# joshspeagle/frankenz

Measured on AMD Instinct MI355X. Metric: object-template likelihood evals/sec (fused fit_predict -> PDFs), higher is better.
Workload: dtype f64 throughout (chi2, ln-likes, every weight, ln-evidence, PDFs; an fp32 estimate of the weight only CLASSIFIES which pairs can matter to an fp64 sum, DESIGN.md 3.1)

## Files before the change

### frankenz_amd/csrc/fz_hist.h

```cpp
#pragma once
#include <type_traits>
#include "fz_kernels.h"
#include "fz_nolist.h"

namespace fz {

#define FZ_HEXP_K 256
#ifndef FZ_HIST_MP
#define FZ_HIST_MP 1
#endif
#ifndef FZ_HIST_TILE384
#define FZ_HIST_TILE384 1
#endif
#ifndef FZ_HIST_REFRESH_TILE
#define FZ_HIST_REFRESH_TILE 1
#endif
#ifndef FZ_HIST_STAGE_LATE
#define FZ_HIST_STAGE_LATE 1
#endif
#ifndef FZ_HIST_SETTLE2
#define FZ_HIST_SETTLE2 0
#endif
#ifndef FZ_HIST_SEG_NW0
#define FZ_HIST_SEG_NW0 16
#endif
#ifndef FZ_HIST_SEG_PFMAX
#define FZ_HIST_SEG_PFMAX 12
#endif
#ifndef FZ_HIST_REFRESH
#define FZ_HIST_REFRESH 32
#endif
#ifndef FZ_HIST_LEAN
#define FZ_HIST_LEAN 1
#endif
#ifndef FZ_HIST_AHEAD
#define FZ_HIST_AHEAD 1
#endif
template <bool L>
__device__ __forceinline__ double fma3(double a, double b, double c) {
    if constexpr (L) { double d; asm("v_fma_f64 %0, %1, %2, %3" : "=v"(d) : "v"(a), "v"(b), "v"(c)); return d; }
    else return fma(a, b, c);
}
template <bool L>
__device__ __forceinline__ double fma3_sb(double a, double b, double c) {
    if constexpr (L) { double d; asm("v_fma_f64 %0, %1, %2, %3" : "=v"(d) : "v"(a), "s"(b), "v"(c)); return d; }
    else return fma(a, b, c);
}
template <bool L>
__device__ __forceinline__ double fma3_mhalf(double a, double c) {
    if constexpr (L) { double d; asm("v_fma_f64 %0, %1, -0.5, %2" : "=v"(d) : "v"(a), "v"(c)); return d; }
    else return fma(a, -0.5, c);
}
template <bool L>
__device__ __forceinline__ int exp_insert(int hi, int n) {
    if constexpr (L) { int r; asm("v_lshl_add_u32 %0, %1, 12, %2" : "=v"(r) : "v"(n & ~(FZ_HEXP_K - 1)), "v"(hi)); return r; }
    else return hi + ((n >> 8) << 20);
}
struct ExpK {
    double c1 = 369.3299304675746;
    double c2 = -0.0027076061740622863;
    double c6 = 1.0 / 6.0;
};
template <bool NEGONLY = false, bool L = false>
__device__ __forceinline__ double exp_small_tab(double x, const double* __restrict__ tab, const ExpK& ek = ExpK()) {
    const double MAGIC = 6755399441055744.0;
    x = NEGONLY ? vmax_raw(x, -700.0) : vmin_raw(vmax_raw(x, -700.0), 700.0);
    const double d = fma(x, ek.c1, MAGIC);
    const double r = fma(d - MAGIC, ek.c2, x);
    const int n = __double2loint(d);
    const double t = tab[n & (FZ_HEXP_K - 1)];
    double p = fma3_sb<L>(r, 1.0 / 120.0, 1.0 / 24.0);
    p = fma3<L>(p, r, ek.c6);
    p = fma(p, r, 0.5);
    p = fma(p, r, 1.0);
    p = fma(p, r, 1.0);
    const double v = t * p;
    static_assert(FZ_HEXP_K == 256, "the exponent insert shifts n by log2 of the table's length");
    return __hiloint2double(exp_insert<L>(__double2hiint(v), n), __double2loint(v));
}

__device__ __forceinline__ double sqrt_nr(double r) {
    const double y = __builtin_amdgcn_rsq(vmax_raw(r, 1e-300));
    const double hy = 0.5 * y;
    double s = r * y;
    s = fma(fma(-s, s, r), hy, s);
    s = fma(fma(-s, s, r), hy, s);
    return s;
}
constexpr double hist_ln(double k) {
    return k == 1.0 ? 0.0 : k == 2.0 ? 0.6931471805599453 : k == 3.0 ? 1.0986122886681098 : k == 4.0 ? 1.3862943611198906
         : k == 5.0 ? 1.6094379124341003 : k == 6.0 ? 1.791759469228055 : k == 7.0 ? 1.9459101090932196 : 2.0794415416798357;
}
template <int WP, bool SMALL = false, bool L = false>
__device__ __forceinline__ double hist_exactw(double c2, const FastTabs& tb, const ExpK& ek = ExpK()) {
    constexpr double K = (double)WP;
    const double r = c2 * (1.0 / K);
    double pw = 1.0;
    if constexpr ((WP >> 1) <= 3) {
        if constexpr ((WP >> 1) >= 1) pw = r;
        if constexpr ((WP >> 1) >= 2) pw = pw * r;
        if constexpr ((WP >> 1) >= 3) pw = pw * r;
    } else {
        double base = r;
#pragma unroll
        for (int e = WP >> 1; e > 0; e >>= 1) { if (e & 1) pw = pw * base; base = base * base; }
    }
    if constexpr (SMALL && (WP >> 1) <= 3) {
        double q = 1.0;
        if constexpr ((WP >> 1) >= 1) q = c2;
        if constexpr ((WP >> 1) >= 2) q = q * c2;
        if constexpr ((WP >> 1) >= 3) q = q * c2;
        if constexpr (WP & 1) {
            const double y = __builtin_amdgcn_rsq(c2), hy = 0.5 * y;
            double sq = c2 * y;
            sq = fma(fma(-sq, sq, c2), hy, sq);
            sq = fma(fma(-sq, sq, c2), hy, sq);
            q = (WP >> 1) ? q * sq : sq;
        }
        constexpr double EK = 0.5 * K - 0.5 * K * hist_ln(K);
        return q * exp_small_tab<true, L>(fma3_mhalf<L>(c2, EK), tb.expt, ek);
    }
    if constexpr (!SMALL && (WP >> 1) <= 3) {
        double q = 1.0;
        if constexpr ((WP >> 1) >= 1) q = c2;
        if constexpr ((WP >> 1) >= 2) q = q * c2;
        if constexpr ((WP >> 1) >= 3) q = q * c2;
        if constexpr (WP & 1) q = (WP >> 1) ? q * sqrt_nr(c2) : sqrt_nr(c2);
        constexpr double EK = 0.5 * K - 0.5 * K * hist_ln(K);
        return q * exp_neg(fma(c2, -0.5, EK), tb);
    }
    if constexpr (WP & 1) pw = pw * sqrt_nr(r);
    const double w = pw * (SMALL ? exp_small_tab(fma(c2, -0.5, 0.5 * K), tb.expt) : exp_clamped(fma(c2, -0.5, 0.5 * K), tb));
    if constexpr ((WP >> 1) > 3) return (c2 < K + 1400.0) ? w : 0.0;
    else return w;
}

template <bool SMALL = false>
__device__ __forceinline__ double hist_exactw_rt(double c2, int wp, const FastTabs& tb) {
    const double K = (double)wp;
    if (wp == 0) return SMALL ? exp_small_tab(-0.5 * c2, tb.expt) : exp_clamped(-0.5 * c2, tb);
    const double r = c2 * rcp_nr<2>(K);
    double pw = 1.0, base = r;
    for (int e = wp >> 1; e > 0; e >>= 1) { if (e & 1) pw = pw * base; base = base * base; }
    if (wp & 1) pw = pw * sqrt_nr(r);
    const double w = pw * (SMALL ? exp_small_tab(fma(c2, -0.5, 0.5 * K), tb.expt) : exp_clamped(fma(c2, -0.5, 0.5 * K), tb));
    return (c2 < K + 1400.0) ? w : 0.0;
}

template <bool SMALL = false>
__device__ __forceinline__ double hist_exactw_rt8(double c2, int wp, double K, double rK, const FastTabs& tb) {
    if (wp == 0) return SMALL ? exp_small_tab<true>(-0.5 * c2, tb.expt) : exp_clamped(-0.5 * c2, tb);
    const double r = c2 * rK, r2 = r * r;
    const int h = wp >> 1;
    double pw = ((h & 1) ? r : 1.0) * ((h & 2) ? r2 : 1.0);
    if (wp & 1) pw = pw * sqrt_nr(r);
    return pw * (SMALL ? exp_small_tab<true>(fma(c2, -0.5, 0.5 * K), tb.expt) : exp_clamped(fma(c2, -0.5, 0.5 * K), tb));
}

template <class SRC>
constexpr int hist_tile() {
    if (FZ_HIST_SETTLE2 && SRC::NB <= 8 && SRC::RW <= 6 && SRC::LMODE == 1) return 128;
    if (FZ_HIST_TILE384 && SRC::NB <= 8 && SRC::RW <= 6) return 384;
    if (SRC::NB <= 8) return (SRC::RW <= 10 && !(SRC::LMODE == 2 && SRC::RW > 6)) ? 256 : 128;
    return SRC::RW <= 18 ? 256 : (SRC::RW <= 34 ? 128 : 64);
}
template <class SRC>
constexpr bool hist_prefetch() {
    if (SRC::NB <= 8) return SRC::NB + SRC::NVAL <= 18;
    return 2 * SRC::NB + 2 * SRC::RW <= 96;
}

__device__ __forceinline__ float wave_maxf_dpp(float v) {
    int x = __float_as_int(v);
    auto mx = [](int a, int b) { float r; asm("v_max_f32 %0, %1, %2" : "=v"(r) : "v"(__int_as_float(a)), "v"(__int_as_float(b))); return __float_as_int(r); };
    x = mx(x, __builtin_amdgcn_update_dpp(x, x, 0xB1, 0xf, 0xf, false));
    x = mx(x, __builtin_amdgcn_update_dpp(x, x, 0x4E, 0xf, 0xf, false));
    x = mx(x, __builtin_amdgcn_update_dpp(x, x, 0x141, 0xf, 0xf, false));
    x = mx(x, __builtin_amdgcn_update_dpp(x, x, 0x140, 0xf, 0xf, false));
    const float a = __int_as_float(__builtin_amdgcn_readlane(x, 0)), b = __int_as_float(__builtin_amdgcn_readlane(x, 16));
    const float c = __int_as_float(__builtin_amdgcn_readlane(x, 32)), d = __int_as_float(__builtin_amdgcn_readlane(x, 48));
    return fmaxf(fmaxf(a, b), fmaxf(c, d));
}

__device__ __forceinline__ double wave_max_pos_hi(double v) {
    int x = __double2hiint(v);
    auto mx = [](int a, int b) { return a > b ? a : b; };
    x = mx(x, __builtin_amdgcn_update_dpp(x, x, 0xB1, 0xf, 0xf, false));
    x = mx(x, __builtin_amdgcn_update_dpp(x, x, 0x4E, 0xf, 0xf, false));
    x = mx(x, __builtin_amdgcn_update_dpp(x, x, 0x141, 0xf, 0xf, false));
    x = mx(x, __builtin_amdgcn_update_dpp(x, x, 0x140, 0xf, 0xf, false));
    const int a = __builtin_amdgcn_readlane(x, 0), b = __builtin_amdgcn_readlane(x, 16), c = __builtin_amdgcn_readlane(x, 32), d = __builtin_amdgcn_readlane(x, 48);
    return __hiloint2double(mx(mx(a, b), mx(c, d)), 0);
}

#ifndef FZ_HIST_CHI2_2OP
#define FZ_HIST_CHI2_2OP 1
#endif
#ifndef FZ_HIST_C2ZERO
#define FZ_HIST_C2ZERO 1e-16
#endif

template <int TW>
struct HistState {
    double S[TW];
    double Sc[TW];
    double wmx[TW];
    float tmax[TW];
    float tthr[TW];
    double wamb[TW];
    int pend[TW];
    int namb[TW];
    int tick, next;
};

template <class SRC>
struct HistArgs {
    SRC src;
    KdeView kv;
    int64_t N;
    double* lmap; double* levid; double* pdfs;
    const int* omap; int* redo; const int* order;
    int normalize;
};
template <class SRC, int TW, int NW, bool EXACT, bool OBJK = (SRC::NB > 8), bool SEG = false>
__global__ __launch_bounds__(NW * 64) void k_hist(HistArgs<SRC> a_, const KdeView* __restrict__ kvp, int acc_stride, int M,
                                                   double wt_thresh, Cand* __restrict__ amb, int64_t cap) {
    constexpr bool LEAN = (FZ_HIST_LEAN == 1) && !SEG;
    constexpr bool AHD = (FZ_HIST_AHEAD == 1) && LEAN && !EXACT && !(FZ_HIST_SETTLE2 == 1) && !OBJK && SRC::RW <= 6;
    auto hq = [&]() -> const HistArgs<SRC>& {
        if constexpr (!LEAN) return a_;
        auto p = __builtin_amdgcn_kernarg_segment_ptr();
        asm volatile("" : "+s"(p));
        return *(const HistArgs<SRC>*)p;
    };
    const int64_t N = a_.N;
    constexpr int TILE = hist_tile<SRC>(), RW = SRC::RW, TDR = RW * TILE, TD = TDR + TILE / 2, NT = NW * 64, OD = SRC::OBJ_DOUBLES;
    constexpr int WP = SRC::WPOW, BT = SRC::NB;
    static_assert(!OBJK || TW == 1, "per-object band counts: one object per wave");
    static_assert(!SEG || (OBJK && SRC::NB <= 8), "segments: run-time band counts, 4-8 bands");
    constexpr double SEG_VBIG = BT <= 5 ? 0x1p192 : (BT == 6 ? 0x1p160 : (BT == 7 ? 0x1p137 : 0x1p120));
    constexpr int KOFF = SRC::LMODE == 2 ? 3 : 2;
    constexpr bool KRT = OBJK;
    int wpr = WP;
    double K = (double)WP;
    bool kok = true;
    double lgq = a_.src.lp.lg_full;
    constexpr int NOBJ = NW * TW;
    constexpr bool S2 = (FZ_HIST_SETTLE2 == 1) && !EXACT && SRC::NB <= 8 && SRC::RW <= 6 && SRC::LMODE == 1;
    constexpr int CAP = S2 ? 192 : 128, DTHR = CAP - 64;
    using tag_t = uint16_t;
    static_assert(WP >= 1 && WP <= 30, "chi2^(1/2) ... chi2^15");
    __shared__ __attribute__((aligned(16))) double tileA[TD];
    __shared__ __attribute__((aligned(16))) double tileB[TD];
    __shared__ __attribute__((aligned(16))) double s_c2[EXACT ? 2 : NOBJ * CAP];
    __shared__ tag_t s_tag[EXACT ? 2 : NOBJ * CAP];
    __shared__ __attribute__((aligned(16))) double s_tabs[EXACT ? FZ_TABS_DOUBLES : FZ_HEXP_K];
    __shared__ __attribute__((aligned(16))) double s_objs[EXACT ? NOBJ * OD : 2];
    __shared__ __attribute__((aligned(16))) double s_obj0[SEG ? NOBJ * OD : 2];
    static_assert(EXACT || TW * OD <= TW * CAP, "an object row must fit its candidate buffer");
    extern __shared__ double s_rows[];
    const int tid = threadIdx.x, lane = tid & 63;
    const int wave = __builtin_amdgcn_readfirstlane(tid >> 6);
    const int64_t nwaves = (int64_t)gridDim.x * NW, gw = (int64_t)blockIdx.x * NW + wave;
    const int64_t ngroups = (N + TW - 1) / TW, nrounds = (ngroups + nwaves - 1) / nwaves;
    const int ntiles = (M + TILE - 1) / TILE;
    SRC src = a_.src;
    src.tb = global_tabs();
    const FastTabs tb = src.tb;
    FastTabs tbx;
    if constexpr (EXACT) tbx = stage_tabs(s_tabs, tid, NT);
    else {
        for (int k = tid; k < FZ_HEXP_K; k += NT) s_tabs[k] = FZ_EXP_TAB[k * (FZ_EXP_K / FZ_HEXP_K)];
        tbx.logt = nullptr; tbx.expt = s_tabs;
    }
    const KdeView kv = [&]() { if constexpr (SEG) return *kvp; else return a_.kv; }();
    const int32_t* posw = SEG ? kv.mc_tag : kv.pos;
    const int w0 = SEG ? 0 : kv.w0;
    double* objs = EXACT ? s_objs + wave * (TW * OD) : s_c2 + wave * (TW * CAP);
    double* obj0 = s_obj0 + (SEG ? wave * (TW * OD) : 0);
    double* rows = s_rows + (size_t)wave * TW * acc_stride;
    double* rc2 = s_c2 + (EXACT ? 0 : wave * (TW * CAP));
    tag_t* rtag = s_tag + (EXACT ? 0 : wave * (TW * CAP));
    Cand* ambw = amb + (size_t)gw * TW * cap;
    auto t_consts = [](double Kd, float& hk23, float& T0c, float& tmarg) {
        const double hk = 0.5 * Kd;
        hk23 = (float)(hk / 8388608.0);
        T0c = (float)((Kd > 0.0 ? -hk * log2(Kd) : 0.0) + Kd * 0.7213475204444817 + hk * (-127.0 + 0.043));
        tmarg = (float)(0.5 + 0.045 * hk);
    };
    float hk23, T0c, tmarg;
    t_consts(K, hk23, T0c, tmarg);
    float tzero = K > 0.0 ? -INFINITY : T0c;
    const float lthr2 = (wt_thresh > 0.0) ? (float)log2(wt_thresh) : -INFINITY;
    int mbits = 0;
    while (((int64_t)1 << mbits) < (int64_t)M) ++mbits;
    const float ldrop0 = fminf(lthr2, -(float)(55 + mbits));
    const double thr_def = wt_thresh * (1.0 + 1e-3);
    auto lnl_c2 = [&](double c2) {
        if constexpr (KRT) return (wpr == 0) ? fma(-0.5, c2, -lgq) : chi2_logpdf<true>(0.5 * K, c2, lgq, tb);
        else return src.lnl_of_chi2(c2);
    };
    double rK = 1.0;
    ExpK ek;
    if constexpr (LEAN) asm volatile("" : "+s"(ek.c1), "+s"(ek.c2), "+v"(ek.c6));
    auto exactw_tab = [&](double c2, const FastTabs& t, auto small) {
        if constexpr (SEG) {
            if constexpr (SRC::LMODE == 2) { if (wpr == WP) return hist_exactw<WP, decltype(small)::value>(c2, t); }
            return hist_exactw_rt8<decltype(small)::value>(c2, wpr, K, rK, t);
        }
        else if constexpr (KRT) return hist_exactw_rt<decltype(small)::value>(c2, wpr, t);
        else return hist_exactw<WP, decltype(small)::value, LEAN>(c2, t, ek);
    };
    double lref = uniform_d(lnl_c2(K));
    auto obj_of = [&](const HistArgs<SRC>& h, int64_t s) -> int64_t {
        if constexpr (!EXACT && !SEG) {
            if (h.order) { const int64_t q = (int64_t)h.order[s]; s = q < 0 ? 0 : (q < h.N ? q : h.N - 1); }
        }
        return h.omap ? (int64_t)h.omap[s] : s;
    };

    for (int64_t rnd = 0; rnd < nrounds; ++rnd) {
        const int64_t g = gw + rnd * nwaves;
        const bool work = g < ngroups;
        const int64_t i0 = work ? g * TW : 0;
        const HistArgs<SRC>& hp = hq();
        [[maybe_unused]] const SRC& srcp = hp.src;
#pragma unroll
        for (int o = 0; o < TW; ++o) {
            const int64_t os = i0 + o < hp.N ? i0 + o : hp.N - 1;
            srcp.park_obj(obj_of(hp, os), objs + o * OD, lane);
        }
        for (int k = lane; k < TW * acc_stride; k += 64) rows[k] = 0.0;
        uint32_t obits = 0; double oslv = 0.0, fk = 1.0; int segcur = -1, ndcur = 0;
        bool segbad = false;
        int nbadm = 0;
        auto seg_lnl = [&](double c2, int nd) {
            const bool dp = src.lp.dim_prior != 0;
            const int wp = dp ? nd - KOFF : 0;
            const double lg = dp ? src.lp.lgtab[nd] : 0.5 * ((double)nd * FZ_LN2PI + oslv);
            const double xl = (wp == 0) ? 0.0 : (0.5 * (double)wp) * log_pos_t<true>(c2, tb);
            return fma(-0.5, c2, xl) - lg;
        };
        if constexpr (SEG) {
            const int64_t os = i0 < hp.N ? i0 : hp.N - 1;
            const int64_t oi = obj_of(hp, os);
            src.park_obj(oi, obj0, lane);
            if constexpr ((SRC::LMODE == 1 || SRC::LMODE == 2) && FZ_HIST_CHI2_2OP && !(SRC::LMODE == 2 && SRC::SAFE)) {
                if (lane < BT) { const double sv = sqrt(obj0[BT + lane]); obj0[BT + lane] = sv; obj0[lane] = obj0[lane] * sv; }
            }
            obits = (uint32_t)__builtin_amdgcn_readfirstlane((int)src.ov.bits[oi]);
            oslv = uniform_d(src.ov.slv[oi]);
            const bool dp = src.lp.dim_prior != 0;
            double lr = -INFINITY; bool bad = false;
            for (int sg = lane; sg < kv.seg_n; sg += 64) {
                const int nd = __popc(obits & kv.seg_mask[sg]);
                const int wp = dp ? nd - KOFF : 0;
                bad |= wp < -1;
                nbadm += (wp == -1) ? kv.seg_start[sg + 1] - kv.seg_start[sg] : 0;
                const double lg = dp ? src.lp.lgtab[nd] : 0.5 * ((double)nd * FZ_LN2PI + oslv);
                const double hw = 0.5 * (double)wp;
                if (wp >= 0) lr = fmax(lr, wp > 0 ? fma(hw, log_pos((double)wp, tb), -hw) - lg : -lg);
            }
            nbadm = __builtin_amdgcn_readfirstlane((int)wave_sum((double)nbadm));
            kok = __ballot(bad) == 0ull && nbadm <= (M >> 3);
            lref = uniform_d(wave_max(lr));
            float h_, t_; t_consts((double)BT, h_, t_, tmarg);
            tmarg = uniform_f(tmarg);
        }
        if constexpr (OBJK && !SEG) {
            const int64_t os = i0 < hp.N ? i0 : hp.N - 1;
            const int64_t oi = obj_of(hp, os);
            const int nb = __builtin_amdgcn_readfirstlane(__popc(srcp.ov.bits[oi]));
            wpr = nb - (SRC::LMODE == 2 ? 3 : 2);
            kok = wpr >= 0;
            if (!kok) wpr = 1;
            const bool dp = src.lp.dim_prior != 0;
            if (!dp) { wpr = 0; kok = true; }
            K = uniform_d((double)wpr);
            t_consts(K, hk23, T0c, tmarg);
            hk23 = uniform_f(hk23); T0c = uniform_f(T0c); tmarg = uniform_f(tmarg);
            tzero = wpr > 0 ? -INFINITY : T0c;
            lgq = uniform_d(dp ? srcp.lp.lgtab[nb] : 0.5 * ((double)nb * FZ_LN2PI + srcp.ov.slv[oi]));
            lref = uniform_d(lnl_c2(K));
        }
        nl_stage_tile<SRC, TILE, NT, true>(src, posw, 0, tileA, tid, wave);
        __syncthreads();
        typename SRC::OR ob[TW];
#pragma unroll
        for (int o = 0; o < TW; ++o) {
            src.load_obj_lds(objs + o * OD, ob[o]);
            if constexpr (BT > 16) {
#pragma unroll
                for (int b = 0; b < BT; ++b) ob[o].x[b] = uniform_d(ob[o].x[b]);
            }
        }
        constexpr bool C2OP = (SRC::LMODE == 1) && FZ_HIST_CHI2_2OP;
        constexpr bool C2OPB = (SRC::LMODE == 2) && !SRC::SAFE && FZ_HIST_CHI2_2OP;
        if constexpr ((C2OP || C2OPB) && !SEG) {
#pragma unroll
            for (int o = 0; o < TW; ++o)
#pragma unroll
                for (int b = 0; b < BT; ++b) {
                    ob[o].v[b] = sqrt(ob[o].v[b]);
                    ob[o].x[b] = ob[o].x[b] * ob[o].v[b];
                    if constexpr (BT > 16) ob[o].x[b] = uniform_d(ob[o].x[b]);
                }
        }
        [[maybe_unused]] const bool mcw = SEG && kv.seg_nrank > 1;
        HistState<TW> hs;
#pragma unroll
        for (int o = 0; o < TW; ++o) {
            hs.S[o] = 0.0; hs.Sc[o] = 0.0; hs.wmx[o] = 0.0;
            hs.tmax[o] = -INFINITY;
            hs.tthr[o] = -INFINITY;
            hs.wamb[o] = 0.0; hs.pend[o] = 0; hs.namb[o] = 0;
        }
        hs.tick = 0; hs.next = 1;

        auto settle = [&](int o, bool act, double c2, int tag, auto badc) {
            double w;
            if (decltype(badc)::value && segbad) w = act ? exp_clamped(seg_lnl(c2, ndcur) - lref, tb) : 0.0;
            else w = act ? exactw_tab(c2, tbx, std::integral_constant<bool, !EXACT>{}) : 0.0;
            if constexpr (SEG) w *= fk;
            hs.Sc[o] += w;
            hs.wmx[o] = vmax_raw(hs.wmx[o], w);
            bool am;
            unsigned long long mask;
            if constexpr (LEAN) {
                const bool stk = w > thr_def, bar = w > hs.wamb[o];
                const unsigned long long mstk = __ballot(stk), mbar = __ballot(bar);
                if (stk) unsafeAtomicAdd(&rows[o * acc_stride + tag + w0], w);
                mask = mbar & ~mstk;
                am = bar && !stk;
            } else {
                if (w > thr_def) unsafeAtomicAdd(&rows[o * acc_stride + tag + w0], w);
                am = act && !(w > thr_def) && w > hs.wamb[o];
                mask = __ballot(am);
            }
            if (mask) {
                const int pre = __builtin_amdgcn_mbcnt_hi((unsigned)(mask >> 32), __builtin_amdgcn_mbcnt_lo((unsigned)mask, 0));
                const int np = __builtin_popcountll(mask);
                if (hs.namb[o] >= 0 && hs.namb[o] + np <= cap) {
                    if (am) { Cand e; e.lnl = c2; e.j = tag; e.pad = SEG ? (ndcur | (mcw ? kv.seg_rank[segcur] << 8 : 0)) : 0; ambw[(size_t)o * cap + hs.namb[o] + pre] = e; }
                    hs.namb[o] += np;
                    if constexpr (SEG) hs.namb[o] = __builtin_amdgcn_readfirstlane(hs.namb[o]);
                } else hs.namb[o] = -1;
            }
        };
        auto drain = [&](int o, auto badc) {
            if constexpr (S2) {
                const int n = hs.pend[o] < 128 ? hs.pend[o] : 128;
                const int rest = hs.pend[o] - n;
                const double ca = rc2[o * CAP + rest + lane], cb = rc2[o * CAP + rest + 64 + lane];
                const int ta = (int)rtag[o * CAP + rest + lane], tb2 = (int)rtag[o * CAP + rest + 64 + lane];
                const bool aa = lane < n, ab = lane + 64 < n;
                double wa, wb;
                if (decltype(badc)::value && segbad) {
                    wa = aa ? exp_clamped(seg_lnl(ca, ndcur) - lref, tb) : 0.0; wb = ab ? exp_clamped(seg_lnl(cb, ndcur) - lref, tb) : 0.0;
                } else {
                    wa = exactw_tab(ca, tbx, std::true_type{}); wb = exactw_tab(cb, tbx, std::true_type{});
                    wa = aa ? wa : 0.0; wb = ab ? wb : 0.0;
                }
                if constexpr (SEG) { wa *= fk; wb *= fk; }
                hs.Sc[o] += wa + wb;
                hs.wmx[o] = vmax_raw(hs.wmx[o], vmax_raw(wa, wb));
                if (wa > thr_def) unsafeAtomicAdd(&rows[o * acc_stride + ta + w0], wa);
                if (wb > thr_def) unsafeAtomicAdd(&rows[o * acc_stride + tb2 + w0], wb);
                const bool ama = aa && !(wa > thr_def) && wa > hs.wamb[o], amb = ab && !(wb > thr_def) && wb > hs.wamb[o];
                const unsigned long long ma = __ballot(ama), mb = __ballot(amb);
                if (ma | mb) {
                    const int na = __builtin_popcountll(ma), nb = __builtin_popcountll(mb);
                    if (hs.namb[o] >= 0 && hs.namb[o] + na + nb <= cap) {
                        const int pa = __builtin_amdgcn_mbcnt_hi((unsigned)(ma >> 32), __builtin_amdgcn_mbcnt_lo((unsigned)ma, 0));
                        const int pb = __builtin_amdgcn_mbcnt_hi((unsigned)(mb >> 32), __builtin_amdgcn_mbcnt_lo((unsigned)mb, 0));
                        if (ama) { Cand e; e.lnl = ca; e.j = ta; e.pad = SEG ? (ndcur | (mcw ? kv.seg_rank[segcur] << 8 : 0)) : 0; ambw[(size_t)o * cap + hs.namb[o] + pa] = e; }
                        if (amb) { Cand e; e.lnl = cb; e.j = tb2; e.pad = SEG ? (ndcur | (mcw ? kv.seg_rank[segcur] << 8 : 0)) : 0; ambw[(size_t)o * cap + hs.namb[o] + na + pb] = e; }
                        hs.namb[o] += na + nb;
                    } else hs.namb[o] = -1;
                }
                hs.pend[o] = rest;
                return;
            }
            const int n = hs.pend[o] < 64 ? hs.pend[o] : 64;
            const int rest = hs.pend[o] - n;
            double c2 = rc2[o * CAP + rest + lane];
            int tag = (int)rtag[o * CAP + rest + lane];
            const bool act = lane < n;
            settle(o, act, c2, tag, badc);
            hs.pend[o] = SEG ? __builtin_amdgcn_readfirstlane(rest) : rest;
        };
        [[maybe_unused]] auto class_flush = [&](int rk, double* row, double* gout) {
            constexpr int NACC = 12;
#if defined(FZ_DIAG_NOFLUSH)
            return;
#endif
            const int G = (int)kv.G, Gp = kv.mc_gp, W0 = kv.mc_w0;
            const int wc = kv.mc_width[rk], w2 = 2 * wc, sh = W0 - wc;
            const double* nt = kv.mc_norm + (size_t)rk * Gp;
            const double* kr = kv.kern + kv.mc_off[rk];
            const double ka = (lane <= w2) ? kr[lane] : 0.0;
            const double kb = (lane + 64 <= w2) ? kr[lane + 64] : 0.0;
            for (int k = lane; k < Gp; k += 64) row[k] = row[k] * nt[k];
            const int kal = __double2loint(ka), kah = __double2hiint(ka), kbl = __double2loint(kb), kbh = __double2hiint(kb);
            const double* r0 = row + sh + NACC * min(lane, (G - 1) / NACC);
            double out[NACC], win[NACC];
#pragma unroll
            for (int a = 0; a < NACC; ++a) { out[a] = 0.0; win[a] = r0[a]; }
            for (int h = 0; h <= w2; h += NACC) {
#pragma unroll
                for (int u = 0; u < NACC; ++u) {
                    if (h + u <= w2) {
                        const int q = w2 - (h + u);
                        const double tap = (q < 64) ? __hiloint2double(__builtin_amdgcn_readlane(kah, q), __builtin_amdgcn_readlane(kal, q))
                                                    : __hiloint2double(__builtin_amdgcn_readlane(kbh, q - 64), __builtin_amdgcn_readlane(kbl, q - 64));
#pragma unroll
                        for (int a = 0; a < NACC; ++a) out[a] = fma(win[(a + u) % NACC], tap, out[a]);
                        win[u] = r0[NACC + h + u];
                    }
                }
            }
            for (int k = lane; k < Gp; k += 64) row[k] = 0.0;
#pragma unroll
            for (int a = 0; a < NACC; ++a) {
                const int t = NACC * lane + a;
                if (t < G) gout[t] = (rk == 0) ? out[a] : gout[t] + out[a];
            }
        };
        auto seg_switch = [&](int sw) {
            constexpr bool UH = SRC::LMODE != 0;
            uint32_t jb = obits & kv.seg_mask[sw & 0x3fff];
            if constexpr (UH) jb = (uint32_t)__builtin_amdgcn_readfirstlane((int)jb);
            const int nd = __popc(jb);
            const bool dp = src.lp.dim_prior != 0;
            wpr = dp ? nd - KOFF : 0;
            if constexpr (UH) wpr = __builtin_amdgcn_readfirstlane(wpr);
            segbad = wpr == -1;
            if (wpr < 0) wpr = 1;
            ndcur = nd;
            K = uniform_d((double)wpr);
            rK = uniform_d(wpr > 0 ? 1.0 / (double)wpr : 1.0);
            static constexpr double LOG2K[9] = {0.0, 0.0, 1.0, 1.5849625007211562, 2.0, 2.321928094887362, 2.584962500721156, 2.807354922057604, 3.0};
            const double hk_ = 0.5 * K, l2k = LOG2K[wpr > 8 ? 8 : wpr];
            hk23 = (float)(hk_ / 8388608.0);
            T0c = (float)(-hk_ * l2k + K * 0.7213475204444817 + hk_ * (-127.0 + 0.043));
            lgq = uniform_d(dp ? src.lp.lgtab[nd] : 0.5 * ((double)nd * FZ_LN2PI + oslv));
            const double dl = uniform_d(fma(hk_, l2k * 0.6931471805599453, -hk_) - lgq) - lref;
            fk = uniform_d(exp_neg(dl, tb));
            hk23 = uniform_f(hk23);
            T0c = uniform_f(T0c + (float)(dl * 1.4426950408889634));
            tzero = wpr > 0 ? -INFINITY : T0c;
            if (segbad) {
                hk23 = 0.f; T0c = -1e30f; tzero = INFINITY; fk = 1.0;
            }
            if constexpr (!EXACT) hs.tthr[0] = segbad ? -INFINITY : wave_maxf_dpp(hs.tmax[0]) + (ldrop0 - 2.f * tmarg);
            src.load_obj_lds(obj0, ob[0]);
#pragma unroll
            for (int b = 0; b < BT; ++b) {
                const bool on = (jb >> b) & 1u;
                if constexpr (SRC::LMODE == 0) ob[0].v[b] = on ? ob[0].v[b] : SEG_VBIG;
                else ob[0].v[b] = on ? ob[0].v[b] : 0.0;
                ob[0].x[b] = on ? ob[0].x[b] : 0.0;
            }
            segcur = UH ? __builtin_amdgcn_readfirstlane(sw & 0x3fff) : (sw & 0x3fff);
        };

        auto pair_chi2 = [&](const typename SRC::MR& mm, const typename SRC::OR& oo) -> double {
                if constexpr (C2OP) {
                    double c = 0.0;
#pragma unroll
                    for (int b = 0; b < BT; ++b) { const double d = fma(-mm.y[b], oo.v[b], oo.x[b]); c = fma(d, d, c); }
                    if constexpr (EXACT) c = (c <= FZ_HIST_C2ZERO) ? 0.0 : c;
                    return c;
                } else if constexpr (C2OPB) {
                    double ys[BT], inter = 0.0, shape = 0.0;
#pragma unroll
                    for (int b = 0; b < BT; ++b) {
                        ys[b] = mm.y[b] * oo.v[b];
                        inter = fma(ys[b], oo.x[b], inter);
                        shape = fma(ys[b], ys[b], shape);
                    }
                    const bool odd = !(shape > 1e-280 && shape < 1e280);
                    const double rc = rcp_nr<1>(shape);
                    double sc = inter * rc;
                    sc = fma(fma(-sc, shape, inter), rc, sc);
                    if (__ballot(odd) != 0ull) {
                        asm volatile("" ::: "memory");
                        if (odd) sc = inter / shape;
                    }
                    double c = 0.0;
#pragma unroll
                    for (int b = 0; b < BT; ++b) { const double d = fma(-sc, ys[b], oo.x[b]); c = fma(d, d, c); }
                    return c;
                } else {
                    double c = src.chi2_of(oo, mm);
                    if constexpr (SEG && SRC::LMODE == 0 && EXACT) c = (c <= FZ_HIST_C2ZERO) ? 0.0 : c;
                    return c;
                }
        };
        if constexpr (SEG) {
            if (kok && nbadm > 0) {
                const bool dp = src.lp.dim_prior != 0;
                double lb = -INFINITY;
                for (int s0 = 0; s0 < kv.seg_n; s0 += 64) {
                    const int sg = s0 + lane;
                    const bool isb = sg < kv.seg_n && dp && (__popc(obits & kv.seg_mask[sg < kv.seg_n ? sg : 0]) - KOFF == -1);
                    unsigned long long bm = __ballot(isb);
                    while (bm) {
                        const int sb = s0 + __builtin_ctzll(bm);
                        bm &= bm - 1;
                        seg_switch(sb);
                        const int j1 = kv.seg_start[sb + 1];
                        for (int j = kv.seg_start[sb] + lane; j < j1; j += 64) {
                            typename SRC::MR mm;
                            src.load_model_rec16(j, mm);
                            double c2 = pair_chi2(mm, ob[0]);
                            if constexpr (C2OP || SRC::LMODE == 0) c2 = (c2 <= FZ_HIST_C2ZERO) ? 0.0 : c2;
                            const double l = seg_lnl(c2, ndcur);
                            lb = fmax(lb, posw[j] < 0 ? -INFINITY : l);
                        }
                    }
                }
                lref = uniform_d(fmax(lref, wave_max(lb)));
                kok = lref < INFINITY;
                segcur = -1;
            }
        }
        auto refresh_bars = [&]() {
#pragma unroll
            for (int o = 0; o < TW; ++o) {
                const float mx = wave_maxf_dpp(hs.tmax[o]);
                hs.tmax[o] = mx;
                hs.tthr[o] = mx + (ldrop0 - 2.f * tmarg);
                if constexpr (SEG) hs.tthr[o] = segbad ? -INFINITY : hs.tthr[o];
                hs.wamb[o] = wave_max_pos_hi(hs.wmx[o]) * (wt_thresh * 0.999);
            }
        };
        constexpr int MP = EXACT ? 1 : FZ_HIST_MP;
        static_assert(!SEG || MP == 1, "segments: one group per trip");
        auto step_body = [&](typename SRC::MR (&m)[MP], int (&ptag)[MP], int st, int t, auto tailc, auto slowc, bool flush) {
            constexpr bool TAIL = decltype(tailc)::value, SLOW = decltype(slowc)::value;
                double c2[MP][TW];
#pragma unroll
                for (int q = 0; q < MP; ++q)
#pragma unroll
                    for (int o = 0; o < TW; ++o) {
                        c2[q][o] = pair_chi2(m[q], ob[o]);
                        if (TAIL) c2[q][o] = (t * TILE + (st + q) * 64 + lane < M) ? c2[q][o] : 1e30;
                    }
                if constexpr (EXACT) {
                    const int j = t * TILE + st * 64 + lane;
#pragma unroll
                    for (int o = 0; o < TW; ++o) {
                        const bool valid = (!TAIL || j < M) && (!SLOW || ptag[0] >= 0);
                        double w;
                        if (SLOW && segbad) w = valid ? exp_clamped(seg_lnl(c2[0][o], ndcur) - lref, tb) : 0.0;
                        else w = valid ? exactw_tab(c2[0][o], tbx, std::false_type{}) : 0.0;
                        if constexpr (SEG) { w *= fk; ptag[0] &= 0xffff; }
                        hs.S[o] += w;
                        hs.Sc[o] = vmax_raw(hs.Sc[o], w);
                        if (w > thr_def) unsafeAtomicAdd(&rows[o * acc_stride + ptag[0] + w0], w);
                        const bool am = valid && !(w > thr_def) && (w >= wt_thresh * 0.999 * hs.Sc[o]);
                        const unsigned long long mask = __ballot(am);
                        if (mask) {
                            const int pre = __builtin_amdgcn_mbcnt_hi((unsigned)(mask >> 32), __builtin_amdgcn_mbcnt_lo((unsigned)mask, 0));
                            const int np = __builtin_popcountll(mask);
                            if (hs.namb[o] >= 0 && hs.namb[o] + np <= cap) {
                                if (am) { Cand e; e.lnl = c2[0][o]; e.j = ptag[0]; e.pad = SEG ? (ndcur | (mcw ? kv.seg_rank[segcur] << 8 : 0)) : 0; ambw[(size_t)o * cap + hs.namb[o] + pre] = e; }
                                hs.namb[o] += np;
                    if constexpr (SEG) hs.namb[o] = __builtin_amdgcn_readfirstlane(hs.namb[o]);
                            } else hs.namb[o] = -1;
                        }
                    }
                    if ((++hs.tick & 15) == 0) {
#pragma unroll
                        for (int o = 0; o < TW; ++o) hs.Sc[o] = wave_max(hs.Sc[o]);
                    }
                } else {
                    float tl[MP][TW];
#pragma unroll
                    for (int q = 0; q < MP; ++q)
#pragma unroll
                        for (int o = 0; o < TW; ++o) {
                            const float cf = (float)c2[q][o];
                            tl[q][o] = fmaf((float)__float_as_int(cf), hk23, fmaf(cf, -0.72134752f, T0c));
                            tl[q][o] = ((C2OP || (SEG && SRC::LMODE == 0)) ? !(cf <= (float)FZ_HIST_C2ZERO) : (cf != 0.f)) ? tl[q][o] : tzero;
                            if (TAIL) tl[q][o] = (t * TILE + (st + q) * 64 + lane < M) ? tl[q][o] : -INFINITY;
                            if constexpr (SLOW) tl[q][o] = (ptag[q] < 0) ? -INFINITY : tl[q][o];
                        }
#pragma unroll
                    for (int q = 0; q < MP; ++q) {
#pragma unroll
                        for (int o = 0; o < TW; ++o) {
                            const bool le = tl[q][o] <= hs.tthr[o];
                            const bool c = !le;
                            asm("v_max_f32 %0, %1, %2" : "=v"(hs.tmax[o]) : "v"(hs.tmax[o]), "v"(tl[q][o]));
                            const unsigned long long mask = __ballot(c);
                            const int slot = __builtin_amdgcn_mbcnt_hi((unsigned)(mask >> 32), __builtin_amdgcn_mbcnt_lo((unsigned)mask, hs.pend[o]));
#if !defined(FZ_DIAG_NOAPPEND)
                            if (c) { rc2[o * CAP + slot] = c2[q][o]; rtag[o * CAP + slot] = (tag_t)ptag[q]; }
#endif
                            hs.pend[o] += __builtin_popcountll(mask);
                            if constexpr (SEG) hs.pend[o] = __builtin_amdgcn_readfirstlane(hs.pend[o]);
                        }
                        if constexpr (!FZ_HIST_REFRESH_TILE) {
                            if (++hs.tick == hs.next) {
                                hs.next = hs.tick < 16 ? 2 * hs.tick : hs.tick + FZ_HIST_REFRESH;
                                refresh_bars();
                            }
                        }
#pragma unroll
                        for (int o = 0; o < TW; ++o) {
#if defined(FZ_DIAG_NODRAIN)
                            if (hs.pend[o] >= DTHR) { hs.pend[o] -= 64; }
#else
                    if constexpr (SLOW) { const int lim = flush ? 1 : DTHR; while (hs.pend[o] >= lim) drain(o, std::true_type{}); }
                    else { while (hs.pend[o] >= DTHR) drain(o, std::false_type{}); }
#endif
                        }
                    }
                }
        };
        auto run_tile = [&](const double* cur, double* nxt, int t, auto tailc, auto slowc) {
            constexpr bool TAIL = decltype(tailc)::value;
            constexpr bool pure = !decltype(slowc)::value;
            constexpr bool LATE = FZ_HIST_STAGE_LATE && pure && hist_prefetch<SRC>() && !(SEG && SRC::NB + SRC::NVAL > FZ_HIST_SEG_PFMAX);
            if (!LATE || !work) { if (t + 1 < ntiles) nl_stage_tile<SRC, TILE, NT, true>(src, posw, t + 1, nxt, tid, wave); }
            if (work) {
                const int32_t* tags = reinterpret_cast<const int32_t*>(cur + TDR);
                static_assert((TILE / 64) % MP == 0, "groups per trip must divide the tile");
                constexpr bool PF = hist_prefetch<SRC>() && !(SEG && SRC::NB + SRC::NVAL > FZ_HIST_SEG_PFMAX);
                if constexpr (pure) {
                    typename SRC::MR mn[PF ? MP : 1];
                    int tagn[MP];
                    if constexpr (PF) {
#pragma unroll
                        for (int q = 0; q < MP; ++q) {
                            src.template load_model_lds<TILE>(cur, q * 64 + lane, mn[q]);
                            tagn[q] = tags[q * 64 + lane];
                        }
                    }
                    if constexpr (LATE) { if (t + 1 < ntiles) nl_stage_tile<SRC, TILE, NT, true>(src, posw, t + 1, nxt, tid, wave); }
#pragma unroll
                    for (int st = 0; st < TILE / 64; st += MP) {
                        typename SRC::MR m[MP];
                        int ptag[MP];
#pragma unroll
                        for (int q = 0; q < MP; ++q) {
                            if constexpr (PF) { m[q] = mn[q]; ptag[q] = tagn[q]; }
                            else { src.template load_model_lds<TILE>(cur, (st + q) * 64 + lane, m[q]); ptag[q] = tags[(st + q) * 64 + lane]; }
                            asm volatile("" : "+v"(ptag[q]));
                        }
                        if (PF && st + MP < TILE / 64) {
#pragma unroll
                            for (int q = 0; q < MP; ++q) {
                                src.template load_model_lds<TILE>(cur, (st + MP + q) * 64 + lane, mn[q]);
                                tagn[q] = tags[(st + MP + q) * 64 + lane];
                            }
                        }
                        if constexpr (AHD && PF) __builtin_amdgcn_sched_barrier(0);
                        step_body(m, ptag, st, t, tailc, std::false_type{}, false);
                    }
                } else {
                    {
#pragma unroll 1
                        for (int st = -1; st < TILE / 64; ++st) {
                            typename SRC::MR m[MP];
                            int ptag[MP];
                            const int stc = st < 0 ? 0 : st;
                            src.template load_model_lds<TILE>(cur, stc * 64 + lane, m[0]);
                            ptag[0] = st < 0 ? (int)0x80000000 : tags[stc * 64 + lane];
                            const int nxt = st + 1 < TILE / 64 ? (tags[(st + 1) * 64] >> 16) & 0x3fff : segcur;
                            if (st >= 0) {
                                const int sw = (__builtin_amdgcn_readfirstlane(ptag[0]) >> 16) & 0x7fff;
                                if ((sw & 0x3fff) != segcur) {
                                    if (mcw && segcur >= 0) {
                                        const int rko = kv.seg_rank[segcur];
                                        if (kv.seg_rank[sw & 0x3fff] != rko) { const HistArgs<SRC>& hc = hq(); class_flush(rko, rows, hc.pdfs + obj_of(hc, i0) * kv.G); }
                                    }
                                    seg_switch(sw);
                                }
                            }
                            const bool flush = __builtin_amdgcn_readfirstlane(nxt) != segcur;
                            step_body(m, ptag, stc, t, tailc, std::true_type{}, flush);
                        }
                    }
                }
                if constexpr (FZ_HIST_REFRESH_TILE && !EXACT) {
                    if (++hs.tick == hs.next) { hs.next = hs.tick < 3 ? hs.tick + 1 : hs.tick + 5; refresh_bars(); }
                }
            }
#if !defined(FZ_DIAG_NOBARRIER)
            __syncthreads();
#endif
        };
        if constexpr (!SEG) {
            for (int t = 0; t < ntiles; t += 2) {
                if (t + 1 < ntiles) run_tile(tileA, tileB, t, std::false_type{}, std::false_type{}); else run_tile(tileA, tileB, t, std::true_type{}, std::false_type{});
                if (t + 1 < ntiles) {
                    if (t + 2 < ntiles) run_tile(tileB, tileA, t + 1, std::false_type{}, std::false_type{}); else run_tile(tileB, tileA, t + 1, std::true_type{}, std::false_type{});
                }
            }
        } else {
            auto tile_pure = [&](const double* cur) -> bool {
                if (!work) return true;
                const int wv = (reinterpret_cast<const int32_t*>(cur + TDR)[(lane % (TILE / 64)) * 64] >> 16) & 0x7fff;
                return __ballot(wv != segcur) == 0ull && !segbad;
            };
            int t = 0;
            while (t < ntiles) {
                if (!(t & 1)) {
                    while (t < ntiles) {
                        if (!tile_pure(tileA)) break;
                        run_tile(tileA, tileB, t, std::false_type{}, std::false_type{}); ++t;
                        if (t >= ntiles || !tile_pure(tileB)) break;
                        run_tile(tileB, tileA, t, std::false_type{}, std::false_type{}); ++t;
                    }
                    if (t >= ntiles) break;
                }
                if (t & 1) run_tile(tileB, tileA, t, std::false_type{}, std::true_type{});
                else run_tile(tileA, tileB, t, std::false_type{}, std::true_type{});
                ++t;
            }
        }

        if (work) {
#pragma unroll 1
            for (int o = 0; o < TW; ++o) {
                const HistArgs<SRC>& hf = hq();
                const KdeView& kvf = SEG ? kv : hf.kv;
                if (i0 + o >= hf.N) break;
                const int64_t i = obj_of(hf, i0 + o);
                double* const pdfs = hf.pdfs;
                auto lnl_fin = [&](double c2) {
                    if constexpr (KRT || !LEAN) return lnl_c2(c2);
                    else return chi2_logpdf<true>(0.5 * WP, c2, hf.src.lp.lg_full, tb);
                };
                double lrf = lref;
                if constexpr (!KRT && LEAN) lrf = uniform_d(lnl_fin(K));
                double* row = rows + o * acc_stride;
                double wbest_run = 0.0;
                if constexpr (!EXACT) {
                    while (hs.pend[o] > 0) drain(o, std::integral_constant<bool, SEG>{});
                } else {
                    wbest_run = wave_max(hs.Sc[o]);
                }
                if constexpr (!EXACT) wbest_run = wave_max(hs.wmx[o]);
                const double lbest = (wbest_run > 0.0) ? uniform_d(lrf + log_pos(wbest_run, tb)) : -INFINITY;
                const double stot = wave_sum(EXACT ? hs.S[o] : hs.Sc[o]);
                const double le = lrf + log_pos(stot, tb);
                const float tm = EXACT ? 0.f : wave_maxf(hs.tmax[o]);
                const bool ok = (le - le == 0.0) && (lbest > -INFINITY) && (EXACT ? (wbest_run > 1e-24) : (tm >= -400.f)) && hs.namb[o] >= 0 && kok;
                if constexpr (SEG) { if (mcw && segcur >= 0) class_flush(kv.seg_rank[segcur], row, pdfs + i * kv.G); }
                const int na = __builtin_amdgcn_readfirstlane(hs.namb[o]);
                if (na > 0) {
                    __builtin_amdgcn_fence(__ATOMIC_RELEASE, "workgroup");
                    __builtin_amdgcn_fence(__ATOMIC_ACQUIRE, "agent");
                    const double thr = wt_thresh * exp_neg(lbest - le, tb);
                    const Cand* cb = ambw + (size_t)o * cap;
                    for (int c0 = 0; c0 < na; c0 += 64) {
                        const int k = c0 + lane;
                        const bool in1 = k < na;
                        const Cand e1 = cb[in1 ? k : 0];
                        double l1, w1;
                        if constexpr (SEG) {
                            l1 = in1 ? seg_lnl(e1.lnl, e1.pad & 0xff) : -INFINITY;
                            w1 = exp_neg(l1 - lref, tb);
                        } else {
                            l1 = in1 ? lnl_fin(e1.lnl) : -INFINITY;
                            w1 = exactw_tab(e1.lnl, tb, std::false_type{});
                        }
                        const bool s1 = in1 && (exp_neg(l1 - le, tb) > thr);
                        if constexpr (SEG) {
                            if (mcw) {
                                if (s1) {
                                    const int rk = e1.pad >> 8, wc = kv.mc_width[rk], p = e1.j - kv.mc_w0;
                                    const double* kr = kv.kern + kv.mc_off[rk];
                                    const double wn = w1 * kv.mc_norm[(size_t)rk * kv.mc_gp + e1.j];
                                    const int G = (int)kv.G;
                                    for (int h = 0; h <= 2 * wc; ++h) {
                                        const int tq = p - wc + h;
                                        if (tq >= 0 && tq < G) unsafeAtomicAdd(&row[tq], wn * kr[h]);
                                    }
                                }
                                continue;
                            }
                        }
                        if (s1) unsafeAtomicAdd(&row[e1.j + w0], w1);
                    }
                }
                if (lane == 0) {
                    if (hf.lmap) hf.lmap[i] = lbest;
                    if (hf.levid) hf.levid[i] = le;
                    if (!ok) hf.redo[1 + atomicAdd(hf.redo, 1)] = (int)i;
                }
                if constexpr (SEG) {
                    if (mcw) {
                        double* gout = pdfs + i * kv.G;
                        const int G = (int)kv.G;
                        if (!ok) { for (int tq = lane; tq < G; tq += 64) gout[tq] = NAN; continue; }
                        double tot = 0.0;
                        for (int tq = lane; tq < G; tq += 64) { const double vq = gout[tq] + row[tq]; row[tq] = vq; tot += vq; }
                        tot = wave_sum(tot);
                        const int normalize = hf.normalize;
                        const double sc = normalize ? 1.0 / tot : 1.0 / stot;
                        for (int tq = lane; tq < G; tq += 64) gout[tq] = normalize ? row[tq] / tot : row[tq] * sc;
                        continue;
                    }
                }
                kde_finalize<true>(kvf, row, ok, hf.normalize, pdfs + i * kvf.G, lane, ok ? 1.0 / stot : 1.0, true);
            }
        }
        __syncthreads();
    }
}

}
```

Baseline: 636.4 billion.

## Prefetch next tile's first model rows across the tile seam before barrier

Moves the end-of-tile barrier into the last pipeline stage so that the first MP model rows and tags of the next LDS tile can be loaded into registers before the current tile's final compute. The next tile's first iteration then takes those rows from carried registers instead of reloading them from LDS, hiding LDS latency at tile boundaries. It also adds an optional early waitcnt knob (off by default) and uses opaque copies of lane/tid to stop the compiler hoisting or rematerialising values. In exchange it holds extra registers live across tiles and adds barrier-placement complexity.

```diff
diff --git a/frankenz_amd/csrc/fz_hist.h b/frankenz_amd/csrc/fz_hist.h
--- a/frankenz_amd/csrc/fz_hist.h
+++ b/frankenz_amd/csrc/fz_hist.h
@@ -35,6 +35,12 @@
 #endif
 #ifndef FZ_HIST_AHEAD
 #define FZ_HIST_AHEAD 1
+#endif
+#ifndef FZ_HIST_WAIT_EARLY
+#define FZ_HIST_WAIT_EARLY 0
+#endif
+#ifndef FZ_HIST_SEAM
+#define FZ_HIST_SEAM 1
 #endif
 template <bool L>
 __device__ __forceinline__ double fma3(double a, double b, double c) {
@@ -227,6 +233,8 @@
                                                    double wt_thresh, Cand* __restrict__ amb, int64_t cap) {
     constexpr bool LEAN = (FZ_HIST_LEAN == 1) && !SEG;
     constexpr bool AHD = (FZ_HIST_AHEAD == 1) && LEAN && !EXACT && !(FZ_HIST_SETTLE2 == 1) && !OBJK && SRC::RW <= 6;
+    constexpr bool WE = (FZ_HIST_WAIT_EARLY == 1) && AHD;
+    constexpr bool SEAM = (FZ_HIST_SEAM == 1) && AHD && hist_prefetch<SRC>() && (FZ_HIST_STAGE_LATE == 1);
     auto hq = [&]() -> const HistArgs<SRC>& {
         if constexpr (!LEAN) return a_;
         auto p = __builtin_amdgcn_kernarg_segment_ptr();
@@ -383,7 +391,9 @@
             lgq = uniform_d(dp ? srcp.lp.lgtab[nb] : 0.5 * ((double)nb * FZ_LN2PI + srcp.ov.slv[oi]));
             lref = uniform_d(lnl_c2(K));
         }
-        nl_stage_tile<SRC, TILE, NT, true>(src, posw, 0, tileA, tid, wave);
+        int tid0 = tid;
+        if constexpr (SEAM) asm volatile("" : "+v"(tid0));
+        nl_stage_tile<SRC, TILE, NT, true>(src, posw, 0, tileA, tid0, wave);
         __syncthreads();
         typename SRC::OR ob[TW];
 #pragma unroll
@@ -447,13 +457,13 @@
                 } else hs.namb[o] = -1;
             }
         };
-        auto drain = [&](int o, auto badc) {
+        auto drain = [&](int o, auto badc, int ln) {
             if constexpr (S2) {
                 const int n = hs.pend[o] < 128 ? hs.pend[o] : 128;
                 const int rest = hs.pend[o] - n;
-                const double ca = rc2[o * CAP + rest + lane], cb = rc2[o * CAP + rest + 64 + lane];
-                const int ta = (int)rtag[o * CAP + rest + lane], tb2 = (int)rtag[o * CAP + rest + 64 + lane];
-                const bool aa = lane < n, ab = lane + 64 < n;
+                const double ca = rc2[o * CAP + rest + ln], cb = rc2[o * CAP + rest + 64 + ln];
+                const int ta = (int)rtag[o * CAP + rest + ln], tb2 = (int)rtag[o * CAP + rest + 64 + ln];
+                const bool aa = ln < n, ab = ln + 64 < n;
                 double wa, wb;
                 if (decltype(badc)::value && segbad) {
                     wa = aa ? exp_clamped(seg_lnl(ca, ndcur) - lref, tb) : 0.0; wb = ab ? exp_clamped(seg_lnl(cb, ndcur) - lref, tb) : 0.0;
@@ -483,9 +493,9 @@
             }
             const int n = hs.pend[o] < 64 ? hs.pend[o] : 64;
             const int rest = hs.pend[o] - n;
-            double c2 = rc2[o * CAP + rest + lane];
-            int tag = (int)rtag[o * CAP + rest + lane];
-            const bool act = lane < n;
+            double c2 = rc2[o * CAP + rest + ln];
+            int tag = (int)rtag[o * CAP + rest + ln];
+            const bool act = ln < n;
             settle(o, act, c2, tag, badc);
             hs.pend[o] = SEG ? __builtin_amdgcn_readfirstlane(rest) : rest;
         };
@@ -694,6 +704,7 @@
                             const bool le = tl[q][o] <= hs.tthr[o];
                             const bool c = !le;
                             asm("v_max_f32 %0, %1, %2" : "=v"(hs.tmax[o]) : "v"(hs.tmax[o]), "v"(tl[q][o]));
+                            if constexpr (WE) { __builtin_amdgcn_sched_barrier(0); __builtin_amdgcn_s_waitcnt(0xc07f); }
                             const unsigned long long mask = __ballot(c);
                             const int slot = __builtin_amdgcn_mbcnt_hi((unsigned)(mask >> 32), __builtin_amdgcn_mbcnt_lo((unsigned)mask, hs.pend[o]));
 #if !defined(FZ_DIAG_NOAPPEND)
@@ -713,13 +724,20 @@
 #if defined(FZ_DIAG_NODRAIN)
                             if (hs.pend[o] >= DTHR) { hs.pend[o] -= 64; }
 #else
-                    if constexpr (SLOW) { const int lim = flush ? 1 : DTHR; while (hs.pend[o] >= lim) drain(o, std::true_type{}); }
-                    else { while (hs.pend[o] >= DTHR) drain(o, std::false_type{}); }
+                    if constexpr (SLOW) { const int lim = flush ? 1 : DTHR; while (hs.pend[o] >= lim) drain(o, std::true_type{}, lane); }
+                    else { while (hs.pend[o] >= DTHR) drain(o, std::false_type{}, lane); }
 #endif
                         }
                     }
                 }
         };
+        auto tile_barrier = [&]() {
+#if !defined(FZ_DIAG_NOBARRIER)
+            __syncthreads();
+#endif
+        };
+        [[maybe_unused]] typename SRC::MR mseam[MP];
+        [[maybe_unused]] int tagseam[MP];
         auto run_tile = [&](const double* cur, double* nxt, int t, auto tailc, auto slowc) {
             constexpr bool TAIL = decltype(tailc)::value;
             constexpr bool pure = !decltype(slowc)::value;
@@ -732,7 +750,10 @@
                 if constexpr (pure) {
                     typename SRC::MR mn[PF ? MP : 1];
                     int tagn[MP];
-                    if constexpr (PF) {
+                    if constexpr (SEAM) {
+#pragma unroll
+                        for (int q = 0; q < MP; ++q) { mn[q] = mseam[q]; tagn[q] = tagseam[q]; }
+                    } else if constexpr (PF) {
 #pragma unroll
                         for (int q = 0; q < MP; ++q) {
                             src.template load_model_lds<TILE>(cur, q * 64 + lane, mn[q]);
@@ -755,6 +776,19 @@
                             for (int q = 0; q < MP; ++q) {
                                 src.template load_model_lds<TILE>(cur, (st + MP + q) * 64 + lane, mn[q]);
                                 tagn[q] = tags[(st + MP + q) * 64 + lane];
+                            }
+                        }
+                        if constexpr (SEAM) {
+                            if (st + MP >= TILE / 64) {
+                                tile_barrier();
+                                if constexpr (!TAIL) {
+                                    const int32_t* tagx = reinterpret_cast<const int32_t*>(nxt + TDR);
+#pragma unroll
+                                    for (int q = 0; q < MP; ++q) {
+                                        src.template load_model_lds<TILE>(nxt, q * 64 + lane, mseam[q]);
+                                        tagseam[q] = tagx[q * 64 + lane];
+                                    }
+                                }
                             }
                         }
                         if constexpr (AHD && PF) __builtin_amdgcn_sched_barrier(0);
@@ -789,10 +823,19 @@
                     if (++hs.tick == hs.next) { hs.next = hs.tick < 3 ? hs.tick + 1 : hs.tick + 5; refresh_bars(); }
                 }
             }
-#if !defined(FZ_DIAG_NOBARRIER)
-            __syncthreads();
-#endif
+            if constexpr (SEAM && pure) { if (!work) tile_barrier(); }
+            else tile_barrier();
         };
+        if constexpr (SEAM) {
+            if (work) {
+                const int32_t* tag0 = reinterpret_cast<const int32_t*>(tileA + TDR);
+#pragma unroll
+                for (int q = 0; q < MP; ++q) {
+                    src.template load_model_lds<TILE>(tileA, q * 64 + lane, mseam[q]);
+                    tagseam[q] = tag0[q * 64 + lane];
+                }
+            }
+        }
         if constexpr (!SEG) {
             for (int t = 0; t < ntiles; t += 2) {
                 if (t + 1 < ntiles) run_tile(tileA, tileB, t, std::false_type{}, std::false_type{}); else run_tile(tileA, tileB, t, std::true_type{}, std::false_type{});
@@ -839,8 +882,10 @@
                 if constexpr (!KRT && LEAN) lrf = uniform_d(lnl_fin(K));
                 double* row = rows + o * acc_stride;
                 double wbest_run = 0.0;
+                int lanef = lane;
+                if constexpr (SEAM) asm volatile("" : "+v"(lanef));
                 if constexpr (!EXACT) {
-                    while (hs.pend[o] > 0) drain(o, std::integral_constant<bool, SEG>{});
+                    while (hs.pend[o] > 0) drain(o, std::integral_constant<bool, SEG>{}, lanef);
                 } else {
                     wbest_run = wave_max(hs.Sc[o]);
                 }
@@ -907,7 +952,7 @@
                         continue;
                     }
                 }
-                kde_finalize<true>(kvf, row, ok, hf.normalize, pdfs + i * kvf.G, lane, ok ? 1.0 / stot : 1.0, true);
+                kde_finalize<true>(kvf, row, ok, hf.normalize, pdfs + i * kvf.G, lanef, ok ? 1.0 / stot : 1.0, true);
             }
         }
         __syncthreads();
```

Result: faster. 657.5 billion, median of 6 (+3.3%).
